# dome272/Paella

Hardware: AMD Instinct MI355X
Metric: images/sec (whole node) + single-image ms, 256x256 @ 8 steps (higher is better)
Workload: dtype f32; 1 GPU; BASELINE configs[1]: Paella 573M-class (stand-in blocks=[4,8,4]) (570.3M params), 32x32 tokens = 256 px, 8 steps, CFG 8.0, CLIP-H-text only (S=4), batch 1 per GPU, + VQGAN f8 decode; denoiser=570m, sample_steps=8, noise=philox, submission=hip-graph replay, world_size_observed=1

## Files before the change

paella_amd/_lib.py:

```python
import ctypes
import os
from ctypes import POINTER, Structure, c_char, c_char_p, c_float, c_int, c_int32, c_int64, c_size_t, c_uint64, c_void_p

_HERE = os.path.dirname(os.path.abspath(__file__))
LIB_PATH = os.path.join(_HERE, "csrc", "libpaella_hip.so")

MAX_LEVELS = 8
MAX_BLOCK_TYPES = 8
ABI_VERSION = 8


class UnetConfig(Structure):
    _fields_ = [
        ("c_in", c_int32), ("c_out", c_int32), ("num_labels", c_int32), ("c_r", c_int32), ("patch_size", c_int32),
        ("c_cond", c_int32), ("n_levels", c_int32),
        ("c_hidden", c_int32 * MAX_LEVELS), ("nhead", c_int32 * MAX_LEVELS), ("blocks", c_int32 * MAX_LEVELS),
        ("level_config", (c_char * MAX_BLOCK_TYPES) * MAX_LEVELS),
        ("clip_embd", c_int32), ("byt5_embd", c_int32), ("clip_seq_len", c_int32), ("kernel_size", c_int32),
        ("self_attn", c_int32),
    ]


class VqganConfig(Structure):
    _fields_ = [
# ... 208 lines not shown
    "paella_test_attention_bf16_ragged": (c_int, [c_void_p, c_void_p, c_void_p, c_void_p, c_void_p, c_void_p, c_int, c_int, c_int, c_int, c_int, c_int, c_void_p,
                                                  c_void_p, c_int, c_void_p]),
    "paella_test_attention_bf16_kw": (c_int, [c_void_p, c_void_p, c_void_p, c_void_p, c_void_p, c_void_p, c_int, c_int, c_int, c_int, c_int, c_int, c_void_p,
                                              c_void_p, c_void_p, c_int, c_void_p]),
    "paella_test_launch_chain": (c_int, [c_void_p, c_int, c_int, c_int, c_void_p]),
    "paella_test_attention_variant": (c_int, [c_int]),
    "paella_test_gemm_dma": (c_int, [c_int]),
    "paella_test_gemm_epi_specialise": (c_int, [c_int]),
    "paella_test_gemm_raster": (c_int, [c_int]),
    "paella_test_gemm_ring": (c_int, [c_int]),
    "paella_test_ring_resident": (ctypes.c_long, [c_int, c_int]),
    "paella_test_gemm_site": (c_int, [c_int, c_int, c_int, c_int, c_int, c_int]),
    "paella_test_gemm_site_cfg": (c_int, [c_int, c_int, c_int, c_int, c_int, c_int, c_int]),
    "paella_test_gemm_big_stagger": (c_int, [c_int]),
    "paella_test_grn_fuse": (c_int, [c_int]),
    "paella_test_ln_fold_ratio": (c_int, [c_float]),
    "paella_test_ln_guard_counter": (c_int, [c_void_p]),
    "paella_test_mlp_grn_fused": (c_int, [c_void_p] * 10 + [c_int, c_int, c_int, c_void_p, c_size_t, c_void_p]),
    "paella_test_gemm_tail_tile": (c_int, [c_int]),
    "paella_test_tail_scores": (c_int, [c_void_p, c_void_p, c_int64, c_int, c_float, c_float, c_float, c_uint64, c_uint64, c_int64, c_void_p, c_void_p]),
    "paella_test_tail_scores_req": (c_int, [c_void_p, c_void_p, c_int64, c_int, c_void_p, c_void_p, c_void_p, c_int, c_uint64, c_void_p, c_void_p]),
    "paella_test_tail_filter_keep": (c_int, [c_void_p, c_void_p, c_int64, c_int, c_float, c_float, c_float, c_int, c_float, c_float, c_int, c_void_p, c_void_p, c_void_p,
                                             c_int, c_void_p, c_void_p, c_void_p, c_void_p, c_void_p]),
    "paella_test_renoise_scores": (c_int, [c_void_p, c_void_p, c_void_p, c_int64, c_int, c_uint64, c_uint64, c_int64, c_float, c_int, c_float, c_void_p, c_void_p, c_void_p,
                                           c_void_p, c_void_p, c_void_p, c_void_p, c_void_p, c_void_p, c_void_p, c_void_p, c_void_p]),
    "paella_test_gemm_prologue": (c_int, [c_void_p, c_void_p, c_void_p, c_int, c_int, c_int, c_int, c_void_p, c_void_p, c_int, c_void_p, c_int, c_int,
                                          c_void_p, c_size_t, c_void_p]),
    "paella_test_gemm_desc": (c_int, [POINTER(TestGemmArgs), c_int, c_int, c_void_p, c_size_t, c_void_p]),
    "paella_test_gemm_args_size": (c_size_t, []),
}
# ... 63 lines not shown
```

paella_amd/csrc/common.h:

```cpp
#pragma once
#include <hip/hip_runtime.h>
#include <stdint.h>
#include <stddef.h>

typedef float f32x4 __attribute__((ext_vector_type(4)));

#define PAELLA_OK 0
#define PAELLA_ERR_ARG -1
#define PAELLA_ERR_HIP -2
#define PAELLA_ERR_WORKSPACE -3
#define PAELLA_ERR_STATE -4

void paella_set_error(const char* fmt, ...);

#define HIP_CHECK_RET(expr)                                                          \
    do {                                                                             \
        hipError_t _e = (expr);                                                      \
        if (_e != hipSuccess) {                                                      \
            paella_set_error("%s:%d: %s -> %s", __FILE__, __LINE__, #expr,           \
                             hipGetErrorString(_e));                                 \
            return PAELLA_ERR_HIP;                                                   \
        }                                                                            \
    } while (0)

// ... 97 lines not shown
    int M, N, K;
    const float* a_scale;
    const float* a_shift;
    int a_rows_per_sample;
    FastDiv a_rps_div;
    const float* grn_gx;
    const float* grn_gamma;
    const float* grn_part;
    int grn_np;
    int force_ring_cfg;
    const float* ln_stats;
    int ln_nblk;
    float ln_eps;
    const float* ln_row;
    float ln_fold_ratio;
    const float* ln_wsum;
    unsigned* ln_guard_count;
    Epilogue ep;
    FusedTail ft;
    ConvGather cv;
    const unsigned short* A16;
    const unsigned short* W16;
    ReqTables rq;
};

struct TailArgs;
static const size_t kGemmMaxTickets = (size_t)1 << 16;
static const size_t kGemmTicketBytes = kGemmMaxTickets * sizeof(unsigned);
int launch_gemm(const GemmArgs& g, void* ws, size_t ws_bytes, hipStream_t stream);
int launch_gemm_cfg(const GemmArgs& g, int cfg, int splitk, void* ws, size_t ws_bytes, hipStream_t stream);
// ... 135 lines not shown
```

paella_amd/csrc/gemm.hip:

```cpp
#include "common.h"
#include "gemm_device.h"
#include "philox.h"
#include <stdio.h>
#include <stdlib.h>
#include "test_hooks.h"
#include <atomic>
#include <mutex>
#include <string>
#include <type_traits>
#include <utility>
#include <vector>

typedef unsigned int u32x4 __attribute__((ext_vector_type(4)));
typedef __bf16 bf16x8 __attribute__((ext_vector_type(8)));

template <typename F, int... Is>
__device__ __forceinline__ void static_for_impl(F& f, std::integer_sequence<int, Is...>) { (f(std::integral_constant<int, Is>{}), ...); }
template <int N, typename F>
__device__ __forceinline__ void static_for(F& f) { static_for_impl(f, std::make_integer_sequence<int, N>{}); }

struct SkPlan {
    int tiles_m, tiles_n;
    int KT;
    unsigned U;
// ... 71 lines not shown
constexpr int tile_wg_per_cu(int WM, int WN, int TM, int TN, int PD, int APRO, bool TAIL, int BK, bool DMA, int RING, bool BF) {
    const int NW = WM * WN, blocks = TM * TN;
    if (RING > 0) {
        const int wish = NW == 8 ? 1 : blocks == 1 ? (RING == 3 ? 5 : 4) : (blocks == 2 ? ((BF && APRO == 2 && TM == 2) ? 3 : 4) : 3);
        const int fit = (160 * 1024) / tile_res(WM, WN, TM, TN, APRO, TAIL, BK, RING).lds_bytes;
        return fit < wish ? (fit < 1 ? 1 : fit) : wish;
    }
    if (TAIL && DMA) return 4;
    if (TAIL && NW == 8 && blocks == 4) return 4;
    if (WM == 2 && WN == 2 && blocks == 1 && PD == 2 && BK == 32 && (APRO == 0 || APRO == 3)) return 5;
    if (DMA && NW == 4 && blocks == 16) return 2;
    if (NW == 8 && WM * TM == 8 && WN * TN == 4 && PD == 2 && BK == 32 && APRO == 0 && !TAIL) return 4;
    return 1;
}

template <int WM, int WN, int TM, int TN, int PD, int APRO, bool TAIL = false, int BK = 32, bool DMA = false, int RING = 0, bool BF = false, int EPI = EPI_RUNTIME, bool REQ = false>
__global__ __launch_bounds__(64 * WM * WN, tile_wg_per_cu(WM, WN, TM, TN, PD, APRO, TAIL, BK, DMA, RING, BF)) void gemm_nt_kernel(GemmArgs g, SkPlan p, float* __restrict__ slabs,
                                                               unsigned* __restrict__ tickets, unsigned slab_bytes) {
    constexpr TileRes RES = tile_res(WM, WN, TM, TN, APRO, TAIL, BK, RING);
    constexpr int BM = RES.BM, BN = RES.BN;
    constexpr int SL = BK / 4;
    constexpr int KG = BK / 16;
    constexpr int NW = WM * WN, NT = 64 * NW;
    constexpr int RP = NT / SL;
    constexpr int LA = (BM * SL + NT - 1) / NT, LB = (BN * SL + NT - 1) / NT;
    static_assert(NW == 4 || NW == 8, "4 or 8 waves per workgroup");
    static_assert(!REQ || TAIL, "the request form exists for the fused tail only");
    static_assert(PD == 1 || PD == 2, "prefetch ring depth 1 or 2");
    static_assert(BK == 32 || BK == 64, "K step of 32 or 64");
    static_assert(!BF || ((DMA || RING > 0) && (APRO == 0 || APRO == 2) && BK == 32), "bf16 operands: direct-to-LDS / ring variants, no operand transform");
    constexpr int ESZ = BF ? 2 : 4;
    constexpr bool DMA_W = DMA || RING > 0, DMA_A = (DMA && (APRO == 0 || APRO == 2)) || RING > 0;
    static_assert(!DMA || (PD == 1 && BK == 32 && (BM * SL) % NT == 0 && (BN * SL) % NT == 0), "DMA variant: 1-deep, K step 32, whole passes");
    constexpr bool PP = RING == 2;
    static_assert(!PP || (BF && NW == 8 && WM == 2 && WN == 4 && TM == 8 && TN == 4 && (APRO == 0 || APRO == 2)), "ping-pong tile: bf16 operands, 2 x 4 waves of 128x64 wave tiles");
    static_assert(RING == 0 || (RING >= 2 && RING <= 4 && !DMA && PD == 1 && BK == 32 && !TAIL && APRO != 3 && (NW == 4 || (TM == 4 && TN == 4 && RING == 3) || PP) && (BM * SL) % NT == 0 && (BN * SL) % NT == 0),
                  "ring variant: 3 or 4 LDS stages (2 for the ping-pong tile), 4 waves (or 8 waves of 64x64 / 128x64 wave tiles), K step 32, whole passes, no implicit convolution");
    static_assert(APRO != 4 || RING > 0, "the GRN-from-raw-statistics prologue exists on ring tiles only");
    constexpr bool BIG = RING > 0 && NW == 8;
    static_assert(!BIG || APRO != 4, "the 8-wave ring tile has no GRN-from-raw-statistics prologue");
    constexpr bool GRN_SIDE = RING > 0 && (APRO == 1 || APRO == 4);
    constexpr bool GRN_FIN = RING > 0 && !BIG;
    constexpr int TILE_FLOATS = RES.tile_floats, STAGE_FLOATS = RES.stage_floats, FLAG_OFF = RES.flag_off, TAIL_FLOATS = RES.tail_floats;
    static_assert(RES.side_samples == (BIG ? 16 : 8) && (RES.grn_scr > 0) == GRN_FIN, "tile_res() and the kernel agree on which ring tiles are BIG");
    __shared__ __attribute__((aligned(16))) float smem[RES.lds_bytes / 4];

    const unsigned G = p.G;
    unsigned gid = blockIdx.x;
    {
        const unsigned q = G >> 3, r = G & 7;
        const unsigned xcd = gid & 7, idx = gid >> 3;
        gid = xcd * q + min(xcd, r) + idx;
    }
    const unsigned u0 = sk_start(p, gid);
    const int n = (int)(p.q + (gid < p.r ? 1u : 0u));
// ... 27 lines not shown
    };
    Stage R[PD];

    int ltile = (int)fast_div(u0, p.dKT);
    int lkt = (int)(u0 - (unsigned)ltile * (unsigned)KT);
    auto rsrc_of = [](const void* ptr, size_t bytes) {
        return __builtin_amdgcn_make_buffer_rsrc(const_cast<void*>(ptr), 0, (int)(bytes > 0xffffffffull ? 0xffffffffull : bytes), 0x00020000);
    };
    const char* const Abase = BF ? reinterpret_cast<const char*>(g.A16) : reinterpret_cast<const char*>(g.A);
    const char* const Wbase = BF ? reinterpret_cast<const char*>(g.W16) : reinterpret_cast<const char*>(g.W);
    const size_t a_bytes = APRO == 3 ? (size_t)(g.M / (g.cv.Ho * g.cv.Wo)) * g.cv.Hi * g.cv.Wi * g.cv.C * sizeof(float)
                                     : ((size_t)(g.M - 1) * g.lda + g.K) * ESZ;
    const size_t w_bytes = ((size_t)(g.N - 1) * g.ldw + g.K) * ESZ;
    __amdgpu_buffer_rsrc_t rsrcA = rsrc_of(Abase, a_bytes), rsrcW = rsrc_of(Wbase, w_bytes);
    __amdgpu_buffer_rsrc_t rsrcS = rsrc_of(g.A, 16);
    const __amdgpu_buffer_rsrc_t rsrcT = rsrc_of((APRO == 1 || APRO == 4) ? g.a_shift : g.A, (APRO == 1 || APRO == 4) ? (size_t)g.K * sizeof(float) : 16);
    const __amdgpu_buffer_rsrc_t rsrcG = rsrc_of(APRO == 4 ? g.grn_gamma : g.A, APRO == 4 ? (size_t)g.K * sizeof(float) : 16);
    unsigned aoff[LA], soff[APRO == 1 ? LA : 1], boff[LB];
    unsigned aux_s_off2 = 0;
    unsigned aux_s_off = 0;
    int cy[APRO == 3 ? LA : 1], cx[APRO == 3 ? LA : 1];
    int ltap = 0, lc0 = 0;
    auto set_tile = [&](int tile) __attribute__((always_inline)) {
        int tile_m, tile_n;
        sk_tile_coords<(BM >= 64)>(p, tile, tile_m, tile_n);
        const int m0 = tile_m * BM, n0 = tile_n * BN;
        size_t a_base;
        int img0 = 0, smp0 = 0;
        if (APRO == 3) {
            img0 = m0 / (g.cv.Ho * g.cv.Wo);
            a_base = (size_t)img0 * g.cv.Hi * g.cv.Wi * g.cv.C * sizeof(float);
// ... 189 lines not shown
                a = __builtin_bit_cast(f32x4, __builtin_shufflevector(lo, hi, 0, 1, 2, 3, 4, 5, 6, 7));
            }
        }
    };
    int kt_cur = 0;

    auto load_unit = [&](Stage& r, int dma_slot) __attribute__((always_inline)) {
        float* dAs = smem + dma_slot * (RING > 0 ? STAGE_FLOATS : TILE_FLOATS) + (wave * (64 / SL)) * BK;
        float* dBs = dAs + BM * BK;
        const int kofs = lkt * (BK * 4);
        if constexpr (RING > 0) {
#pragma unroll
            for (int i = 0; i < LA; ++i) dma_b128_to_lds(rsrcA, dAs + i * RP * BK, aoff[i], kofs);
#pragma unroll
            for (int i = 0; i < LB; ++i) dma_b128_to_lds<((BIG || TM * TN != 1) ? 0 : PAELLA_RING_W_AUX)>(rsrcW, dBs + i * RP * BK, boff[i], kofs);
            if (GRN_SIDE && wave == NW - 1) {
                float* dX = smem + dma_slot * STAGE_FLOATS + TILE_FLOATS;
                if (BIG) {
                    if (lane_k < 8) dma_b128_to_lds(rsrcT, dX, (unsigned)(lane_k * 16), kofs);
                    dma_b128_to_lds(rsrcS, dX + 64, aux_s_off, kofs);
                    dma_b128_to_lds(rsrcS, dX + 64 + 256, aux_s_off2, kofs);
                } else if (APRO == 4) {
                    if (lane_k < 8) {
                        dma_b128_to_lds(rsrcT, dX, (unsigned)(lane_k * 16), kofs);
                        dma_b128_to_lds(rsrcG, dX + 32, (unsigned)(lane_k * 16), kofs);
                    }
                    dma_b128_to_lds(rsrcS, dX + 64, aux_s_off, kofs);
                } else {
                    dma_b128_to_lds(rsrcT, dX, (unsigned)((lane_k & 7) * 16), kofs);
                    dma_b128_to_lds(rsrcS, dX + 256, aux_s_off, kofs);
                }
            }
            return;
        }
        int oy = 0, ox = 0;
        if (APRO == 3) {
            oy = g.cv.oy0 + g.cv.tsign * (ltap >> g.cv.tw_log2);
            ox = g.cv.ox0 + g.cv.tsign * (ltap & ((1 << g.cv.tw_log2) - 1));
        }
#pragma unroll
        for (int i = 0; i < LA; ++i) {
            if (APRO == 3) {
                const int yy = cy[i] + oy, xx = cx[i] + ox;
                r.ok[i] = (unsigned)yy < (unsigned)g.cv.Hi && (unsigned)xx < (unsigned)g.cv.Wi;
// ... 486 lines not shown
                    const int row = (wn * TN + j) * 16 + r16;
                    bf[kk][j] = *reinterpret_cast<const f32x4*>(Bs + row * BK + ((c4 ^ (row & (SL - 1))) << 2));
                }
            }
            if (APRO == 2 && ln_any) {
#pragma unroll
                for (int kk = 0; kk < KG; ++kk)
#pragma unroll
                    for (int i = 0; i < TM; ++i) ln_fix(af[kk][i], i, BF_FIX ? kt_ring * BK + (kk * 4 + kq) * 4 : 0);
            }
            if (APRO == 1) {
                const float* X = Bs + BN * BK;
#pragma unroll
                for (int kk = 0; kk < KG; ++kk) {
                    const int c4 = kk * 4 + kq;
                    const f32x4 t = *reinterpret_cast<const f32x4*>(X + c4 * 4);
#pragma unroll
                    for (int i = 0; i < TM; ++i) {
                        const f32x4 sc = *reinterpret_cast<const f32x4*>(X + 256 + sidx[i] * 32 + c4 * 4);
                        af[kk][i] = af[kk][i] * sc + t;
                    }
                }
            }
            if (APRO == 4) {
                const float* X = Bs + BN * BK;
#pragma unroll
                for (int kk = 0; kk < KG; ++kk) {
                    const int c4 = kk * 4 + kq;
                    const f32x4 t = *reinterpret_cast<const f32x4*>(X + c4 * 4);
                    const f32x4 gm = *reinterpret_cast<const f32x4*>(X + 32 + c4 * 4);
#pragma unroll
                    for (int i = 0; i < TM; ++i) {
                        const f32x4 gx = *reinterpret_cast<const f32x4*>(X + 64 + sidx[i] * 32 + c4 * 4);
                        const f32x4 sc = gm * gx * rinv[i] + 1.0f;
                        af[kk][i] = af[kk][i] * sc + t;
                    }
                }
            }
            if constexpr (BF) {
                if (TM * TN == 1) {
#pragma unroll
                    for (int kk = 0; kk < KG; kk += 2) {
                        acc[0][0] = mma_bf16(bf[kk][0], af[kk][0], acc[0][0]);
                        acc2 = mma_bf16(bf[kk + 1][0], af[kk + 1][0], acc2);
                    }
                } else {
#pragma unroll
                    for (int kk = 0; kk < KG; ++kk)
#pragma unroll
                        for (int i = 0; i < TM; ++i)
// ... 19 lines not shown
                            for (int j = 0; j < TN; ++j)
                                acc[i][j] = __builtin_amdgcn_mfma_f32_16x16x4f32(bf[kk][j][e], af[kk][i][e], acc[i][j], 0, 0, 0);
            }
        };
        auto fetch_ring = [&](int stage) __attribute__((always_inline)) {
            load_unit(R[0], stage);
            if (++loaded < n) {
                if (++lkt == KT) {
                    lkt = 0;
                    ++ltile;
                    set_tile(ltile);
                }
            }
        };
        constexpr int PER_UNIT = LA + LB;
        constexpr int SIDE_DMAS = (APRO == 4 || BIG) ? 3 : 2;
        if constexpr (PP) {
            using I0 = std::integral_constant<int, 0>;
            using I1 = std::integral_constant<int, 1>;
            using I2 = std::integral_constant<int, 2>;
            using I3 = std::integral_constant<int, 3>;
            using I4 = std::integral_constant<int, 4>;
            int lbuf = 0;
            auto pp_issue = [&](auto sec_tag) __attribute__((always_inline)) {
                constexpr int sec = decltype(sec_tag)::value;
                float* dAs = smem + lbuf * STAGE_FLOATS + (wave * (64 / SL)) * BK;
                float* dBs = dAs + BM * BK;
                const int kofs = lkt * (BK * 4);
                if constexpr (sec == 0) {
                    dma_b128_to_lds(rsrcA, dAs, aoff[0], kofs);
                    dma_b128_to_lds(rsrcA, dAs + 2 * RP * BK, aoff[2], kofs);
// ... 193 lines not shown
                __builtin_amdgcn_sched_barrier(0);
                if (i + seg_len == n) asm volatile("s_waitcnt vmcnt(0)" ::: "memory");
                if (first_seg) ln_row_stats();
                flush(ctile, ckt, ckt + seg_len, first_seg);
                first_seg = false;
                i += seg_len;
                ckt += seg_len;
                if (ckt == KT) { ckt = 0; ++ctile; }
            }
            return;
        }
        for (int i = 0; i < n;) {
            const int seg_len = min(KT - ckt, n - i);
            enter_tile(ctile);
            for (int s2 = 0; s2 < seg_len; ++s2) {
                if (GRN_SIDE && wave == NW - 1) asm volatile("s_waitcnt vmcnt(%0)" ::"n"((RING - 2) * (PER_UNIT + SIDE_DMAS)) : "memory");
                else asm volatile("s_waitcnt vmcnt(%0)" ::"n"((RING - 2) * PER_UNIT) : "memory");
                __builtin_amdgcn_s_barrier();
                asm volatile("" ::: "memory");
                fetch_ring(ls);
                __builtin_amdgcn_sched_barrier(0);
                compute_ring(cs, ckt + s2);
                __builtin_amdgcn_sched_barrier(0);
                cs = cs + 1 == RING ? 0 : cs + 1;
                ls = ls + 1 == RING ? 0 : ls + 1;
            }
            if (i + seg_len == n) asm volatile("s_waitcnt vmcnt(0)" ::: "memory");
            flush(ctile, ckt, ckt + seg_len, first_seg);
            first_seg = false;
            i += seg_len;
            ckt += seg_len;
// ... 193 lines not shown
};
template <int APRO> struct RingEpi { using set = EpiSet<>; };
template <> struct RingEpi<0> { using set = EpiSet<EPI_B, EPI_BGF, EPI_BGS, EPI_BR, EPI_BRS>; };
template <> struct RingEpi<1> { using set = EpiSet<EPI_BR, EPI_BRS, EPI_BRT, EPI_BRST>; };
template <> struct RingEpi<2> { using set = EpiSet<EPI_B>; };
template <> struct RingEpi<4> { using set = EpiSet<EPI_BR, EPI_BRS, EPI_BRT, EPI_BRST>; };

struct Launch {
    const GemmArgs& g;
    const SkPlan& p;
    float* slabs;
    unsigned* tickets;
    unsigned slab_bytes;
    hipStream_t st;
};
template <int ID, int APRO, bool TAIL = false, bool DMA = false, int RING = 0, bool BF = false, int EPI = EPI_RUNTIME, bool REQ = false>
static void launch_kernel(const Launch& l) {
    constexpr Tile t = kCfgs[ID];
    hipLaunchKernelGGL((gemm_nt_kernel<t.wm, t.wn, t.tm, t.tn, t.pd, APRO, TAIL, t.bk, DMA, RING, BF, EPI, REQ>), dim3(l.p.G), dim3(64 * t.waves()), 0, l.st, l.g, l.p, l.slabs,
                       l.tickets, l.slab_bytes);
}

template <int ID, int APRO, int EPI>
static bool launch_ring_if(int cls, const Launch& l) {
    if (cls != EPI) return false;
    launch_kernel<ID, APRO, false, false, kCfgs[ID].ring, false, EPI>(l);
    g_last_epi = EPI;
    return true;
}
template <int ID, int APRO, int... C>
static void launch_ring_epi(EpiSet<C...>, const Launch& l) {
    const int cls = g_gemm_epi_spec ? epi_class(l.g) : EPI_RUNTIME;
    if (!(launch_ring_if<ID, APRO, C>(cls, l) || ...)) launch_ring_if<ID, APRO, EPI_RUNTIME>(EPI_RUNTIME, l);
}
template <int ID, int APRO>
static void launch_ring_apro(const Launch& l) {
    using set = typename std::conditional<kCfgs[ID].tm * kCfgs[ID].tn == 1, typename RingEpi<APRO>::set, EpiSet<>>::type;
    launch_ring_epi<ID, APRO>(set{}, l);
}
template <int ID>
static void launch_ring(const Launch& l) {
    if (l.g.grn_gx) launch_ring_apro<ID, 4>(l);
    else if (l.g.a_scale) launch_ring_apro<ID, 1>(l);
    else if (l.g.ln_stats) launch_ring_apro<ID, 2>(l);
    else launch_ring_apro<ID, 0>(l);
}

template <int ID>
static void launch_one(const Launch& l) {
    constexpr Tile t = kCfgs[ID];
    const GemmArgs& g = l.g;
    if constexpr (t.has(V_DMA | V_DMA_PLAIN)) {
        if (g_gemm_dma && g.K % t.bk == 0 && !g.cv.enabled && !g.a_scale && !g.ln_stats) return launch_kernel<ID, 0, false, true>(l);
// ... 284 lines not shown
    g_prof.shape.insert(g_prof.shape.end(), shp, shp + 5);
    return rc;
}

static std::atomic<float> g_ln_fold_ratio{kLnFoldMaxRatio};
extern "C" int paella_test_ln_fold_ratio(float ratio) { g_ln_fold_ratio = ratio; return PAELLA_OK; }
static std::atomic<unsigned*> g_ln_guard_count{nullptr};
extern "C" int paella_test_ln_guard_counter(unsigned* dev_word) { g_ln_guard_count = dev_word; return PAELLA_OK; }

int launch_gemm_cfg(const GemmArgs& g_in, int cfg, int splitk, void* ws, size_t ws_bytes, hipStream_t st) {
    GemmArgs g = g_in;
    g.ln_fold_ratio = g_ln_fold_ratio.load(std::memory_order_relaxed);
    g.ln_guard_count = g_ln_guard_count.load(std::memory_order_relaxed);
    g.a_rps_div = fast_div_of((unsigned)(g.a_rows_per_sample > 0 ? g.a_rows_per_sample : 1));
    g.ep.rps_div = fast_div_of((unsigned)(g.ep.rows_per_sample > 0 ? g.ep.rows_per_sample : 1));
    return prof_bracket(g, st, true, [&]() { return launch_gemm_cfg_impl(g, cfg, splitk, ws, ws_bytes, st); });
}

extern "C" int paella_prof_enable(int on) {
    std::lock_guard<std::mutex> lock(g_prof_mu);
    g_prof.on = on != 0;
    g_prof.used = 0;
    g_prof.flops.clear();
    g_prof.bytes.clear();
    g_prof.shape.clear();
    g_prof.epi.clear();
    g_prof.grid.clear();
    return PAELLA_OK;
}

// ... 149 lines not shown
        if (bf && cfg_has(cfg, V_BF16) && g.ln_stats && !g.ln_row && !prepass_fits && bf16_ln_needs_prepass(cfg, g.A != nullptr)) {
            cfg = 18;
            if (splitk >= 0) G = (unsigned)(tiles_of_cfg(cfg, g.M, g.N) * (splitk < 1 ? 1 : splitk));
        }
    }
    const Tile& tc = kCfgs[cfg];
    const int BM = tc.res().BM, BN = tc.res().BN;
    g_last_cfg = cfg;
    if (bf && g.ln_stats && !g.ln_row && bf16_ln_needs_prepass(cfg, g.A != nullptr)) {
        if (!prepass_fits) { paella_set_error("internal: bf16 LayerNorm-consuming launch on tile %d without room for its row pre-pass", cfg); return PAELLA_ERR_STATE; }
        const int rc = ln_prepass();
        if (rc != PAELLA_OK) return rc;
    }
    if (bf && !cfg_has(cfg, V_BF16)) { paella_set_error("gemm: tile config %d has no bf16-operand variant (%s do)", cfg, ids_with(V_BF16).c_str()); return PAELLA_ERR_ARG; }
    if ((g.grn_gx || g.ep.grn_gx_out) && (!tc.ring || tc.waves() == 8)) { paella_set_error("gemm: the in-epilogue / on-load GRN statistics need a ring tile (got tile %d)", cfg); return PAELLA_ERR_STATE; }
    if (g.grn_gx && (!g.grn_gamma || !g.a_shift || !g.grn_part || g.grn_np <= 0 || g.a_scale || g.ln_stats || g.a_rows_per_sample % 16)) {
        paella_set_error("gemm: bad GRN-from-statistics operand description"); return PAELLA_ERR_ARG;
    }
    if (g.ep.grn_gx_out && (!g.ep.grn_part_out || !(g.ep.grn_rps == 16 || g.ep.grn_rps == BM) || g.M % g.ep.grn_rps ||
                            g.ep.grn_np != ((g.N + BN - 1) / BN) * tc.wn)) {
        paella_set_error("gemm: in-epilogue GRN needs tiles that cover whole samples (rows per sample 16 or %d, got %d) and grn_np = tiles_n * %d", BM, g.ep.grn_rps, tc.wn);
        return PAELLA_ERR_ARG;
    }
    if (tc.ring && !ring_ok(g, cfg)) { paella_set_error("gemm: tile config %d (LDS-DMA ring) needs K %% 32 == 0, no implicit convolution and <= 8 samples per tile", cfg); return PAELLA_ERR_ARG; }
    SkPlan p;
    unsigned slab_bytes = 0;
    const int rc = make_plan("gemm", g, cfg, bf, G, g_gemm_big_stagger.load(std::memory_order_relaxed), have_ws, slab_cap, p, slab_bytes);
    if (rc != PAELLA_OK) return rc;
    const Launch l{g, p, have_ws ? reinterpret_cast<float*>(reinterpret_cast<char*>(ws) + kGemmTicketBytes) : nullptr, have_ws ? reinterpret_cast<unsigned*>(ws) : nullptr, slab_bytes, st};
    if (!launch_tile(TileIds{}, cfg, bf, l)) { paella_set_error("gemm: tile config %d (%dx%d) exists for bf16 operands only", cfg, BM, BN); return PAELLA_ERR_ARG; }
    LAUNCH_CHECK_RET();
// ... 80 lines not shown
```

paella_amd/csrc/internal.h:

```cpp
#pragma once
#include "common.h"
#include "../../include/paella_hip.h"
#include <vector>

#define RET_IF(expr)                      \
    do {                                  \
        int _rc = (expr);                 \
        if (_rc != PAELLA_OK) return _rc; \
    } while (0)

struct DevBuf {
    float* p = nullptr;
    size_t n = 0;
    bool loaded = false;
};
int devbuf_alloc(DevBuf& b, size_t n);
struct DevBuf16 {
    unsigned short* p = nullptr;
    size_t n = 0;
};

struct Arena {
    char* base;
    size_t cap, off;
// ... 34 lines not shown
    return t;
}
static inline paella_tail_args tail_block_stream(const float* logits_c, const float* logits_u, int64_t rows, int L, const float* cfg_pairs, const float* temperature,
                                                 const uint64_t* seeds, int rows_per_sample, const int* step, const float* t_next, const int* active, const int64_t* init_noise,
                                                 const int64_t* pin_keep, const int64_t* pin_tokens, const int* pin_on, int64_t* tokens_out, int64_t* sampled_out) {
    paella_tail_args t = {};
    t.logits_c = logits_c; t.logits_u = logits_u; t.rows = rows; t.L = L; t.cfg_pairs = cfg_pairs; t.temperature_tab = temperature; t.seeds = seeds;
    t.rows_per_sample = rows_per_sample; t.step = step; t.t_next_tab = t_next; t.active = active; t.init_noise = init_noise;
    t.pin_keep = pin_keep; t.pin_tokens = pin_tokens; t.pin_on = pin_on; t.tokens_out = tokens_out; t.sampled_out = sampled_out;
    return t;
}

static inline GemmArgs gemm_args(const float* A, int lda, const float* Wt, int ldw, float* C, int ldc, int M, int N, int K) {
    GemmArgs g;
    g.A = A; g.lda = lda; g.W = Wt; g.ldw = ldw; g.C = C; g.ldc = ldc; g.M = M; g.N = N; g.K = K;
    g.a_scale = nullptr; g.a_shift = nullptr; g.a_rows_per_sample = 1; g.a_rps_div.mul = 0; g.a_rps_div.shr = 0; g.a_rps_div.pass = 0xffffffffu; g.grn_gx = nullptr; g.grn_gamma = nullptr; g.grn_part = nullptr; g.grn_np = 0; g.force_ring_cfg = 0; g.ln_stats = nullptr; g.ln_nblk = 0; g.ln_eps = 1e-6f; g.ln_wsum = nullptr; g.ln_row = nullptr; g.ln_fold_ratio = 4.0f; g.ln_guard_count = nullptr;
    g.ep = make_epilogue();
    g.ft.temperature = 1.f; g.ft.mode = 0; g.ft.seed = 0; g.ft.seed_ptr = nullptr; g.ft.offset = 0; g.ft.row_offset = 0; g.ft.row_offset_ptr = nullptr;
    g.ft.part_score = nullptr; g.ft.part_idx = nullptr;
    g.cv.enabled = 0;
    g.A16 = nullptr; g.W16 = nullptr;
    return g;
}
```

paella_amd/csrc/model.hip:

```cpp
#include "internal.h"
#include "test_hooks.h"
#include "../../include/paella_hip.h"

#include <math.h>
#include <stdarg.h>
#include <stdio.h>
#include <string.h>

#include <map>
#include <string>
#include <vector>

static thread_local char g_err[2048] = "";
void paella_set_error(const char* fmt, ...) {
    va_list ap;
    va_start(ap, fmt);
    vsnprintf(g_err, sizeof(g_err), fmt, ap);
    va_end(ap);
}
extern "C" const char* paella_last_error(void) { return g_err; }
extern "C" int paella_abi_version(void) { return PAELLA_ABI_VERSION; }

int devbuf_alloc(DevBuf& b, size_t n) {
    if (b.p && b.n == n) return PAELLA_OK;
// ... 22 lines not shown
    int fused_ts = -1;
    int attn_index = -1;
    bool emit_rowstat = false;
    bool ln_from_stats = false;
    int c_from = 0, c_to = 0;
};

struct paella_unet {
    paella_unet_config cfg;
    std::vector<Block> down, up;
    std::map<std::string, TensorSpec> specs;
    std::map<std::string, DevBuf> t;
    DevBuf ts_w, ts_b, freqs;
    DevBuf kv_w, kv_b;
    std::map<std::string, DevBuf> wsum;
    int precision = 0;
    std::map<std::string, DevBuf16> t16;
    std::map<std::string, DevBuf> wsum16;
    std::vector<int> kv_col;
    int kv_total = 0;
    int ts_total = 0;
    int n_attn = 0;
    std::vector<int> attn_c;
    bool finalized = false;
    bool freqs_set = false;
    bool clf_from_stats = false;
    int c_max = 0;
};

static const float* T(const paella_unet* m, const std::string& k) {
// ... 168 lines not shown
    if (rc != PAELLA_OK) { delete m; return rc; }
    if (m->ts_total > 0) {
        rc = devbuf_alloc(m->ts_w, (size_t)m->ts_total * cfg->c_r);
        if (rc == PAELLA_OK) rc = devbuf_alloc(m->ts_b, (size_t)m->ts_total);
        if (rc != PAELLA_OK) { delete m; return rc; }
    }
    *out = m;
    return PAELLA_OK;
}

extern "C" void paella_unet_destroy(paella_unet* m) {
    if (!m) return;
    for (auto& kv : m->t) if (kv.second.p) (void)hipFree(kv.second.p);
    for (auto& kv : m->wsum) if (kv.second.p) (void)hipFree(kv.second.p);
    for (auto& kv : m->wsum16) if (kv.second.p) (void)hipFree(kv.second.p);
    for (auto& kv : m->t16) if (kv.second.p) (void)hipFree(kv.second.p);
    if (m->kv_w.p) (void)hipFree(m->kv_w.p);
    if (m->kv_b.p) (void)hipFree(m->kv_b.p);
    if (m->ts_w.p) (void)hipFree(m->ts_w.p);
    if (m->ts_b.p) (void)hipFree(m->ts_b.p);
    if (m->freqs.p) (void)hipFree(m->freqs.p);
    delete m;
}

int repack_into(Repack kind, const float* src, const std::vector<int64_t>& shape, DevBuf& dst, hipStream_t st) {
    int64_t numel = 1;
    for (int64_t d : shape) numel *= d;
    switch (kind) {
        case RP_COPY:
            RET_IF(devbuf_alloc(dst, numel));
// ... 128 lines not shown
        RET_IF(devbuf_alloc(dst, (size_t)t.second.first));
        RET_IF(launch_rowsum_bf16(it->second.p, dst.p, t.second.first, t.second.second, st));
    }
    HIP_CHECK_RET(hipStreamSynchronize(st));
    return PAELLA_OK;
}

extern "C" int paella_unet_set_precision(paella_unet* m, int mode, void* stream) {
    if (!m) { paella_set_error("null argument"); return PAELLA_ERR_ARG; }
    if (mode != 0 && mode != 1) { paella_set_error("precision mode must be 0 (fp32) or 1 (bf16 operands)"); return PAELLA_ERR_ARG; }
    m->precision = mode;
    if (mode == 1 && m->finalized) return make_shadows(m, (hipStream_t)stream);
    return PAELLA_OK;
}
extern "C" int paella_unet_get_precision(const paella_unet* m) { return m ? m->precision : 0; }

extern "C" int paella_unet_finalize(paella_unet* m, void* stream) {
    if (!m) { paella_set_error("null argument"); return PAELLA_ERR_ARG; }
    for (auto& kv : m->specs) {
        auto it = m->t.find(kv.first);
        if (it == m->t.end() || !it->second.loaded) { paella_set_error("tensor '%s' was never loaded", kv.first.c_str()); return PAELLA_ERR_STATE; }
    }
    {
        hipStream_t st = (hipStream_t)stream;
        std::vector<std::pair<std::string, std::pair<int, int>>> todo;
        auto want = [&](const Block& b) {
            if (b.type == BT_ATTN && b.ln_from_stats) todo.push_back({b.prefix + ".attention.attn.in_proj_weight", {3 * b.c, b.c}});
            if (b.type == BT_UP && b.ln_from_stats) todo.push_back({b.prefix + ".1.weight", {4 * b.c_to, b.c_from}});
        };
        for (const Block& b : m->down) want(b);
// ... 41 lines not shown
            const int perm[2] = {1, 0};
            RET_IF(launch_permute(T(m, b.prefix + ".kv_mapper.1.weight"), wkv_t.p, shp, perm, 2, st));
            GemmArgs g = gemm_args(win, ch, wkv_t.p, ch, m->kv_w.p + (size_t)m->kv_col[b.attn_index] * cc, cc, 2 * ch, cc, ch);
            RET_IF(launch_gemm_cfg(g, 18, 1, nullptr, 0, st));
            GemmArgs gb = gemm_args(T(m, b.prefix + ".kv_mapper.1.bias"), ch, win, ch, m->kv_b.p + m->kv_col[b.attn_index], 2 * ch, 1, 2 * ch, ch);
            gb.ep.bias = bin;
            RET_IF(launch_gemm_cfg(gb, 5, 1, nullptr, 0, st));
            return PAELLA_OK;
        };
        if (rc == PAELLA_OK) for (const Block& b : m->down) { rc = compose(b); if (rc != PAELLA_OK) break; }
        if (rc == PAELLA_OK) for (const Block& b : m->up) { rc = compose(b); if (rc != PAELLA_OK) break; }
        if (hipStreamSynchronize(st) != hipSuccess && rc == PAELLA_OK) { paella_set_error("finalize: stream error while composing the conditioning projections"); rc = PAELLA_ERR_HIP; }
        if (wkv_t.p) (void)hipFree(wkv_t.p);
        if (rc != PAELLA_OK) return rc;
    }
    if (!m->freqs_set) {
        const int half = m->cfg.c_r / 2;
        std::vector<float> f(half > 0 ? half : 1);
        const float e = logf(10000.0f) / (float)(half - 1);
        for (int k = 0; k < half; ++k) f[k] = expf((float)k * -e);
        RET_IF(paella_unet_set_timestep_freqs(m, f.data(), half));
    }
    m->finalized = true;
    if (m->precision == 1) RET_IF(make_shadows(m, (hipStream_t)stream));
    return PAELLA_OK;
}

extern "C" size_t paella_unet_cond_bytes(const paella_unet* m, int B, int S) {
    if (!m) return 0;
    const size_t n = (size_t)B * S * (size_t)m->kv_total;
// ... 204 lines not shown
        g2.A16 = cx.f.g16; g2.W16 = w2_16;
        g2.ep.bias = T(m, b.prefix + ".channelwise.4.bias");
        g2.ep.residual = x; g2.ep.ldr = ch;
        g2.ep.c16 = x16;
        if (b.emit_rowstat) g2.ep.rowstat_out = cx.f.rowstat;
        if (b.fused_ts >= 0) {
            g2.ep.ts = cx.f.ts + b.fused_ts; g2.ep.ts_stride = m->ts_total; g2.ep.rows_per_sample = rps;
        }
        RET_IF(launch_gemm(g2, cx.f.splitk, kSplitKBudget, cx.st));
        return PAELLA_OK;
    }
    if (b.type == BT_RES)
        RET_IF(launch_dwconv_ln(x, skip, T(m, b.prefix + ".depthwise.weight"), T(m, b.prefix + ".depthwise.bias"), cx.f.h, cx.B, h, w, ch, 1e-6f, cx.st));
    else
        RET_IF(launch_layernorm(x, cx.f.h, rows, ch, 1e-6f, 1.f, 0.f, 0, 0, 0, cx.st));
    GemmArgs g1 = gemm_args(cx.f.h, ch, T(m, b.prefix + ".channelwise.0.weight"), ch, cx.f.g, 4 * ch, (int)rows, 4 * ch, ch);
    g1.ep.bias = T(m, b.prefix + ".channelwise.0.bias");
    g1.ep.act = ACT_GELU;
    const int fused_tile = (rps % 16 == 0 && m->precision == 0) ? gemm_grn_fused_tile((int)rows, 4 * ch, ch, rps, false) : 0;
    if (fused_tile) {
        const int np = (4 * ch / 32) * 2;
        g1.ep.grn_gx_out = cx.f.grn_scale; g1.ep.grn_part_out = cx.f.grn_gx; g1.ep.grn_rps = rps; g1.ep.grn_np = np;
        g1.force_ring_cfg = fused_tile;
        RET_IF(launch_gemm(g1, cx.f.splitk, kSplitKBudget, cx.st));
        GemmArgs g2 = gemm_args(cx.f.g, 4 * ch, T(m, b.prefix + ".channelwise.4.weight"), 4 * ch, x, ch, (int)rows, ch, 4 * ch);
        g2.grn_gx = cx.f.grn_scale; g2.grn_part = cx.f.grn_gx; g2.grn_np = np; g2.grn_gamma = T(m, b.prefix + ".channelwise.2.gamma");
        g2.a_shift = T(m, b.prefix + ".channelwise.2.beta");
        g2.a_rows_per_sample = rps;
        g2.ep.bias = T(m, b.prefix + ".channelwise.4.bias");
        g2.ep.residual = x; g2.ep.ldr = ch;
        if (b.emit_rowstat) g2.ep.rowstat_out = cx.f.rowstat;
        if (b.fused_ts >= 0) {
            g2.ep.ts = cx.f.ts + b.fused_ts; g2.ep.ts_stride = m->ts_total; g2.ep.rows_per_sample = rps;
        }
        RET_IF(launch_gemm(g2, cx.f.splitk, kSplitKBudget, cx.st));
        return PAELLA_OK;
    }
    if (rps % 16 == 0) {
        g1.ep.sumsq_out = cx.f.grn_gx;
        RET_IF(launch_gemm(g1, cx.f.splitk, kSplitKBudget, cx.st));
        RET_IF(launch_grn_from_partials(cx.f.grn_gx, T(m, b.prefix + ".channelwise.2.gamma"), cx.f.grn_scale, cx.B, rps / 16, 4 * ch, cx.st));
    } else {
        RET_IF(launch_gemm(g1, cx.f.splitk, kSplitKBudget, cx.st));
        RET_IF(launch_grn_scale(cx.f.g, T(m, b.prefix + ".channelwise.2.gamma"), cx.f.grn_scale, cx.f.grn_gx, cx.B, rps, 4 * ch, cx.st));
    }
    GemmArgs g2 = gemm_args(cx.f.g, 4 * ch, T(m, b.prefix + ".channelwise.4.weight"), 4 * ch, x, ch, (int)rows, ch, 4 * ch);
    g2.a_scale = cx.f.grn_scale;
    g2.a_shift = T(m, b.prefix + ".channelwise.2.beta");
    g2.a_rows_per_sample = rps;
    g2.ep.bias = T(m, b.prefix + ".channelwise.4.bias");
    g2.ep.residual = x; g2.ep.ldr = ch;
    g2.ep.c16 = x16;
    if (b.emit_rowstat) g2.ep.rowstat_out = cx.f.rowstat;
    if (b.fused_ts >= 0) {
        g2.ep.ts = cx.f.ts + b.fused_ts; g2.ep.ts_stride = m->ts_total; g2.ep.rows_per_sample = rps;
    }
    RET_IF(launch_gemm(g2, cx.f.splitk, kSplitKBudget, cx.st));
    return PAELLA_OK;
}

static int run_attn_block(FwdCtx& cx, const Block& b, float* x, int h, int w) {
    const paella_unet* m = cx.m;
    const int ch = b.c;
    const int64_t rows = (int64_t)cx.B * h * w;
    const int nh = m->cfg.nhead[b.level];
// ... 701 lines not shown
```

Baseline: 47.19 images/sec.

## Fold GRN beta shift into second MLP GEMM bias at finalize

```diff
diff --git a/paella_amd/_lib.py b/paella_amd/_lib.py
--- a/paella_amd/_lib.py
+++ b/paella_amd/_lib.py
@@ -246,6 +246,9 @@
     "paella_test_gemm_site_cfg": (c_int, [c_int, c_int, c_int, c_int, c_int, c_int, c_int]),
     "paella_test_gemm_big_stagger": (c_int, [c_int]),
     "paella_test_grn_fuse": (c_int, [c_int]),
+    "paella_test_grn_shift_fold": (c_int, [c_int]),
+    "paella_test_gemm_noshift": (c_int, [c_int]),
+    "paella_test_gemm_noshift_launches": (c_int64, []),
     "paella_test_ln_fold_ratio": (c_int, [c_float]),
     "paella_test_ln_guard_counter": (c_int, [c_void_p]),
     "paella_test_mlp_grn_fused": (c_int, [c_void_p] * 10 + [c_int, c_int, c_int, c_void_p, c_size_t, c_void_p]),
diff --git a/paella_amd/csrc/common.h b/paella_amd/csrc/common.h
--- a/paella_amd/csrc/common.h
+++ b/paella_amd/csrc/common.h
@@ -135,6 +135,7 @@
     float ln_eps;
     const float* ln_row;
     float ln_fold_ratio;
+    unsigned a_shift_bytes;
     const float* ln_wsum;
     unsigned* ln_guard_count;
     Epilogue ep;
diff --git a/paella_amd/csrc/gemm.hip b/paella_amd/csrc/gemm.hip
--- a/paella_amd/csrc/gemm.hip
+++ b/paella_amd/csrc/gemm.hip
@@ -109,7 +109,7 @@
     return 1;
 }
 
-template <int WM, int WN, int TM, int TN, int PD, int APRO, bool TAIL = false, int BK = 32, bool DMA = false, int RING = 0, bool BF = false, int EPI = EPI_RUNTIME, bool REQ = false>
+template <int WM, int WN, int TM, int TN, int PD, int APRO, bool TAIL = false, int BK = 32, bool DMA = false, int RING = 0, bool BF = false, int EPI = EPI_RUNTIME, bool REQ = false, bool NOSHIFT = false>
 __global__ __launch_bounds__(64 * WM * WN, tile_wg_per_cu(WM, WN, TM, TN, PD, APRO, TAIL, BK, DMA, RING, BF)) void gemm_nt_kernel(GemmArgs g, SkPlan p, float* __restrict__ slabs,
                                                                unsigned* __restrict__ tickets, unsigned slab_bytes) {
     constexpr TileRes RES = tile_res(WM, WN, TM, TN, APRO, TAIL, BK, RING);
@@ -134,6 +134,9 @@
     static_assert(APRO != 4 || RING > 0, "the GRN-from-raw-statistics prologue exists on ring tiles only");
     constexpr bool BIG = RING > 0 && NW == 8;
     static_assert(!BIG || APRO != 4, "the 8-wave ring tile has no GRN-from-raw-statistics prologue");
+    static_assert(!NOSHIFT || (RING > 0 && !BIG && (APRO == 1 || APRO == 4)), "the shift-free form exists for the GRN prologues of the 4-wave ring tiles");
+    constexpr bool SIDE_SPREAD = NOSHIFT && APRO == 4;
+    constexpr bool SHIFT = (APRO == 1 || APRO == 4) && !NOSHIFT;
     constexpr bool GRN_SIDE = RING > 0 && (APRO == 1 || APRO == 4);
     constexpr bool GRN_FIN = RING > 0 && !BIG;
     constexpr int TILE_FLOATS = RES.tile_floats, STAGE_FLOATS = RES.stage_floats, FLAG_OFF = RES.flag_off, TAIL_FLOATS = RES.tail_floats;
@@ -191,7 +194,7 @@
     const size_t w_bytes = ((size_t)(g.N - 1) * g.ldw + g.K) * ESZ;
     __amdgpu_buffer_rsrc_t rsrcA = rsrc_of(Abase, a_bytes), rsrcW = rsrc_of(Wbase, w_bytes);
     __amdgpu_buffer_rsrc_t rsrcS = rsrc_of(g.A, 16);
-    const __amdgpu_buffer_rsrc_t rsrcT = rsrc_of((APRO == 1 || APRO == 4) ? g.a_shift : g.A, (APRO == 1 || APRO == 4) ? (size_t)g.K * sizeof(float) : 16);
+    const __amdgpu_buffer_rsrc_t rsrcT = rsrc_of(SHIFT ? g.a_shift : g.A, !SHIFT ? 16 : APRO == 1 ? (size_t)g.a_shift_bytes : (size_t)g.K * sizeof(float));
     const __amdgpu_buffer_rsrc_t rsrcG = rsrc_of(APRO == 4 ? g.grn_gamma : g.A, APRO == 4 ? (size_t)g.K * sizeof(float) : 16);
     unsigned aoff[LA], soff[APRO == 1 ? LA : 1], boff[LB];
     unsigned aux_s_off2 = 0;
@@ -411,7 +414,13 @@
             for (int i = 0; i < LA; ++i) dma_b128_to_lds(rsrcA, dAs + i * RP * BK, aoff[i], kofs);
 #pragma unroll
             for (int i = 0; i < LB; ++i) dma_b128_to_lds<((BIG || TM * TN != 1) ? 0 : PAELLA_RING_W_AUX)>(rsrcW, dBs + i * RP * BK, boff[i], kofs);
-            if (GRN_SIDE && wave == NW - 1) {
+            if constexpr (SIDE_SPREAD) {
+                float* dX = smem + dma_slot * STAGE_FLOATS + TILE_FLOATS;
+                if (wave == NW - 2) {
+                    if (lane_k < 8) dma_b128_to_lds(rsrcG, dX + 32, (unsigned)(lane_k * 16), kofs);
+                }
+                if (wave == NW - 1) dma_b128_to_lds(rsrcS, dX + 64, aux_s_off, kofs);
+            } else if (GRN_SIDE && wave == NW - 1) {
                 float* dX = smem + dma_slot * STAGE_FLOATS + TILE_FLOATS;
                 if (BIG) {
                     if (lane_k < 8) dma_b128_to_lds(rsrcT, dX, (unsigned)(lane_k * 16), kofs);
@@ -419,12 +428,12 @@
                     dma_b128_to_lds(rsrcS, dX + 64 + 256, aux_s_off2, kofs);
                 } else if (APRO == 4) {
                     if (lane_k < 8) {
-                        dma_b128_to_lds(rsrcT, dX, (unsigned)(lane_k * 16), kofs);
+                        if (!NOSHIFT) dma_b128_to_lds(rsrcT, dX, (unsigned)(lane_k * 16), kofs);
                         dma_b128_to_lds(rsrcG, dX + 32, (unsigned)(lane_k * 16), kofs);
                     }
                     dma_b128_to_lds(rsrcS, dX + 64, aux_s_off, kofs);
                 } else {
-                    dma_b128_to_lds(rsrcT, dX, (unsigned)((lane_k & 7) * 16), kofs);
+                    if (!NOSHIFT) dma_b128_to_lds(rsrcT, dX, (unsigned)((lane_k & 7) * 16), kofs);
                     dma_b128_to_lds(rsrcS, dX + 256, aux_s_off, kofs);
                 }
             }
@@ -941,11 +950,13 @@
 #pragma unroll
                 for (int kk = 0; kk < KG; ++kk) {
                     const int c4 = kk * 4 + kq;
-                    const f32x4 t = *reinterpret_cast<const f32x4*>(X + c4 * 4);
+                    f32x4 t;
+                    if constexpr (!NOSHIFT) t = *reinterpret_cast<const f32x4*>(X + c4 * 4);
 #pragma unroll
                     for (int i = 0; i < TM; ++i) {
                         const f32x4 sc = *reinterpret_cast<const f32x4*>(X + 256 + sidx[i] * 32 + c4 * 4);
-                        af[kk][i] = af[kk][i] * sc + t;
+                        if constexpr (NOSHIFT) af[kk][i] = af[kk][i] * sc;
+                        else af[kk][i] = af[kk][i] * sc + t;
                     }
                 }
             }
@@ -954,13 +965,15 @@
 #pragma unroll
                 for (int kk = 0; kk < KG; ++kk) {
                     const int c4 = kk * 4 + kq;
-                    const f32x4 t = *reinterpret_cast<const f32x4*>(X + c4 * 4);
+                    f32x4 t;
+                    if constexpr (!NOSHIFT) t = *reinterpret_cast<const f32x4*>(X + c4 * 4);
                     const f32x4 gm = *reinterpret_cast<const f32x4*>(X + 32 + c4 * 4);
 #pragma unroll
                     for (int i = 0; i < TM; ++i) {
                         const f32x4 gx = *reinterpret_cast<const f32x4*>(X + 64 + sidx[i] * 32 + c4 * 4);
                         const f32x4 sc = gm * gx * rinv[i] + 1.0f;
-                        af[kk][i] = af[kk][i] * sc + t;
+                        if constexpr (NOSHIFT) af[kk][i] = af[kk][i] * sc;
+                        else af[kk][i] = af[kk][i] * sc + t;
                     }
                 }
             }
@@ -1010,7 +1023,7 @@
             }
         };
         constexpr int PER_UNIT = LA + LB;
-        constexpr int SIDE_DMAS = (APRO == 4 || BIG) ? 3 : 2;
+        constexpr int SIDE_DMAS = ((APRO == 4 || BIG) ? 3 : 2) - (NOSHIFT ? 1 : 0);
         if constexpr (PP) {
             using I0 = std::integral_constant<int, 0>;
             using I1 = std::integral_constant<int, 1>;
@@ -1234,7 +1247,8 @@
             const int seg_len = min(KT - ckt, n - i);
             enter_tile(ctile);
             for (int s2 = 0; s2 < seg_len; ++s2) {
-                if (GRN_SIDE && wave == NW - 1) asm volatile("s_waitcnt vmcnt(%0)" ::"n"((RING - 2) * (PER_UNIT + SIDE_DMAS)) : "memory");
+                if (SIDE_SPREAD && wave >= NW - 2) asm volatile("s_waitcnt vmcnt(%0)" ::"n"((RING - 2) * (PER_UNIT + 1)) : "memory");
+                else if (!SIDE_SPREAD && GRN_SIDE && wave == NW - 1) asm volatile("s_waitcnt vmcnt(%0)" ::"n"((RING - 2) * (PER_UNIT + SIDE_DMAS)) : "memory");
                 else asm volatile("s_waitcnt vmcnt(%0)" ::"n"((RING - 2) * PER_UNIT) : "memory");
                 __builtin_amdgcn_s_barrier();
                 asm volatile("" ::: "memory");
@@ -1458,29 +1472,41 @@
     unsigned slab_bytes;
     hipStream_t st;
 };
-template <int ID, int APRO, bool TAIL = false, bool DMA = false, int RING = 0, bool BF = false, int EPI = EPI_RUNTIME, bool REQ = false>
+template <int ID, int APRO, bool TAIL = false, bool DMA = false, int RING = 0, bool BF = false, int EPI = EPI_RUNTIME, bool REQ = false, bool NOSHIFT = false>
 static void launch_kernel(const Launch& l) {
     constexpr Tile t = kCfgs[ID];
-    hipLaunchKernelGGL((gemm_nt_kernel<t.wm, t.wn, t.tm, t.tn, t.pd, APRO, TAIL, t.bk, DMA, RING, BF, EPI, REQ>), dim3(l.p.G), dim3(64 * t.waves()), 0, l.st, l.g, l.p, l.slabs,
+    hipLaunchKernelGGL((gemm_nt_kernel<t.wm, t.wn, t.tm, t.tn, t.pd, APRO, TAIL, t.bk, DMA, RING, BF, EPI, REQ, NOSHIFT>), dim3(l.p.G), dim3(64 * t.waves()), 0, l.st, l.g, l.p, l.slabs,
                        l.tickets, l.slab_bytes);
 }
 
-template <int ID, int APRO, int EPI>
+static std::atomic<int> g_gemm_noshift{1};
+static std::atomic<long long> g_gemm_noshift_launches{0};
+extern "C" int paella_test_gemm_noshift(int on) { g_gemm_noshift = on != 0; return PAELLA_OK; }
+extern "C" long long paella_test_gemm_noshift_launches(void) { return g_gemm_noshift_launches.load(); }
+
+template <int ID, int APRO, int EPI, bool NOSHIFT>
 static bool launch_ring_if(int cls, const Launch& l) {
     if (cls != EPI) return false;
-    launch_kernel<ID, APRO, false, false, kCfgs[ID].ring, false, EPI>(l);
+    launch_kernel<ID, APRO, false, false, kCfgs[ID].ring, false, EPI, false, NOSHIFT>(l);
     g_last_epi = EPI;
+    if (NOSHIFT) ++g_gemm_noshift_launches;
     return true;
 }
-template <int ID, int APRO, int... C>
+template <int ID, int APRO, bool NOSHIFT, int... C>
 static void launch_ring_epi(EpiSet<C...>, const Launch& l) {
     const int cls = g_gemm_epi_spec ? epi_class(l.g) : EPI_RUNTIME;
-    if (!(launch_ring_if<ID, APRO, C>(cls, l) || ...)) launch_ring_if<ID, APRO, EPI_RUNTIME>(EPI_RUNTIME, l);
+    if (!(launch_ring_if<ID, APRO, C, NOSHIFT>(cls, l) || ...)) launch_ring_if<ID, APRO, EPI_RUNTIME, NOSHIFT>(EPI_RUNTIME, l);
 }
 template <int ID, int APRO>
 static void launch_ring_apro(const Launch& l) {
-    using set = typename std::conditional<kCfgs[ID].tm * kCfgs[ID].tn == 1, typename RingEpi<APRO>::set, EpiSet<>>::type;
-    launch_ring_epi<ID, APRO>(set{}, l);
+    constexpr bool small = kCfgs[ID].tm * kCfgs[ID].tn == 1;
+    using set = typename std::conditional<small, typename RingEpi<APRO>::set, EpiSet<>>::type;
+    if constexpr (APRO == 4) {
+        if (!l.g.a_shift_bytes) return launch_ring_epi<ID, APRO, true>(set{}, l);
+    } else if constexpr (small && APRO == 1) {
+        if (!l.g.a_shift_bytes && g_gemm_noshift) return launch_ring_epi<ID, APRO, true>(set{}, l);
+    }
+    launch_ring_epi<ID, APRO, false>(set{}, l);
 }
 template <int ID>
 static void launch_ring(const Launch& l) {
@@ -1795,6 +1821,8 @@
     g.ln_guard_count = g_ln_guard_count.load(std::memory_order_relaxed);
     g.a_rps_div = fast_div_of((unsigned)(g.a_rows_per_sample > 0 ? g.a_rows_per_sample : 1));
     g.ep.rps_div = fast_div_of((unsigned)(g.ep.rows_per_sample > 0 ? g.ep.rows_per_sample : 1));
+    g.a_shift_bytes = g.a_shift ? (unsigned)g.K * (unsigned)sizeof(float) : 0u;
+    if (!g.a_shift) g.a_shift = g.A;
     return prof_bracket(g, st, true, [&]() { return launch_gemm_cfg_impl(g, cfg, splitk, ws, ws_bytes, st); });
 }
 
@@ -1974,7 +2002,7 @@
     }
     if (bf && !cfg_has(cfg, V_BF16)) { paella_set_error("gemm: tile config %d has no bf16-operand variant (%s do)", cfg, ids_with(V_BF16).c_str()); return PAELLA_ERR_ARG; }
     if ((g.grn_gx || g.ep.grn_gx_out) && (!tc.ring || tc.waves() == 8)) { paella_set_error("gemm: the in-epilogue / on-load GRN statistics need a ring tile (got tile %d)", cfg); return PAELLA_ERR_STATE; }
-    if (g.grn_gx && (!g.grn_gamma || !g.a_shift || !g.grn_part || g.grn_np <= 0 || g.a_scale || g.ln_stats || g.a_rows_per_sample % 16)) {
+    if (g.grn_gx && (!g.grn_gamma || !g.grn_part || g.grn_np <= 0 || g.a_scale || g.ln_stats || g.a_rows_per_sample % 16)) {
         paella_set_error("gemm: bad GRN-from-statistics operand description"); return PAELLA_ERR_ARG;
     }
     if (g.ep.grn_gx_out && (!g.ep.grn_part_out || !(g.ep.grn_rps == 16 || g.ep.grn_rps == BM) || g.M % g.ep.grn_rps ||
diff --git a/paella_amd/csrc/internal.h b/paella_amd/csrc/internal.h
--- a/paella_amd/csrc/internal.h
+++ b/paella_amd/csrc/internal.h
@@ -72,7 +72,7 @@
 static inline GemmArgs gemm_args(const float* A, int lda, const float* Wt, int ldw, float* C, int ldc, int M, int N, int K) {
     GemmArgs g;
     g.A = A; g.lda = lda; g.W = Wt; g.ldw = ldw; g.C = C; g.ldc = ldc; g.M = M; g.N = N; g.K = K;
-    g.a_scale = nullptr; g.a_shift = nullptr; g.a_rows_per_sample = 1; g.a_rps_div.mul = 0; g.a_rps_div.shr = 0; g.a_rps_div.pass = 0xffffffffu; g.grn_gx = nullptr; g.grn_gamma = nullptr; g.grn_part = nullptr; g.grn_np = 0; g.force_ring_cfg = 0; g.ln_stats = nullptr; g.ln_nblk = 0; g.ln_eps = 1e-6f; g.ln_wsum = nullptr; g.ln_row = nullptr; g.ln_fold_ratio = 4.0f; g.ln_guard_count = nullptr;
+    g.a_scale = nullptr; g.a_shift = nullptr; g.a_shift_bytes = 0; g.a_rows_per_sample = 1; g.a_rps_div.mul = 0; g.a_rps_div.shr = 0; g.a_rps_div.pass = 0xffffffffu; g.grn_gx = nullptr; g.grn_gamma = nullptr; g.grn_part = nullptr; g.grn_np = 0; g.force_ring_cfg = 0; g.ln_stats = nullptr; g.ln_nblk = 0; g.ln_eps = 1e-6f; g.ln_wsum = nullptr; g.ln_row = nullptr; g.ln_fold_ratio = 4.0f; g.ln_guard_count = nullptr;
     g.ep = make_epilogue();
     g.ft.temperature = 1.f; g.ft.mode = 0; g.ft.seed = 0; g.ft.seed_ptr = nullptr; g.ft.offset = 0; g.ft.row_offset = 0; g.ft.row_offset_ptr = nullptr;
     g.ft.part_score = nullptr; g.ft.part_idx = nullptr;
diff --git a/paella_amd/csrc/model.hip b/paella_amd/csrc/model.hip
--- a/paella_amd/csrc/model.hip
+++ b/paella_amd/csrc/model.hip
@@ -7,6 +7,7 @@
 #include <stdio.h>
 #include <string.h>
 
+#include <atomic>
 #include <map>
 #include <string>
 #include <vector>
@@ -60,6 +61,8 @@
     DevBuf ts_w, ts_b, freqs;
     DevBuf kv_w, kv_b;
     std::map<std::string, DevBuf> wsum;
+    std::map<std::string, DevBuf> b2f;
+    bool grn_shift_fold = true;
     int precision = 0;
     std::map<std::string, DevBuf16> t16;
     std::map<std::string, DevBuf> wsum16;
@@ -258,6 +261,7 @@
     for (auto& kv : m->t) if (kv.second.p) (void)hipFree(kv.second.p);
     for (auto& kv : m->wsum) if (kv.second.p) (void)hipFree(kv.second.p);
     for (auto& kv : m->wsum16) if (kv.second.p) (void)hipFree(kv.second.p);
+    for (auto& kv : m->b2f) if (kv.second.p) (void)hipFree(kv.second.p);
     for (auto& kv : m->t16) if (kv.second.p) (void)hipFree(kv.second.p);
     if (m->kv_w.p) (void)hipFree(m->kv_w.p);
     if (m->kv_b.p) (void)hipFree(m->kv_b.p);
@@ -416,6 +420,9 @@
     return PAELLA_OK;
 }
 extern "C" int paella_unet_get_precision(const paella_unet* m) { return m ? m->precision : 0; }
+
+static std::atomic<int> g_grn_shift_fold{1};
+extern "C" int paella_test_grn_shift_fold(int on) { g_grn_shift_fold = on != 0; return PAELLA_OK; }
 
 extern "C" int paella_unet_finalize(paella_unet* m, void* stream) {
     if (!m) { paella_set_error("null argument"); return PAELLA_ERR_ARG; }
@@ -487,6 +494,24 @@
         if (wkv_t.p) (void)hipFree(wkv_t.p);
         if (rc != PAELLA_OK) return rc;
     }
+    {
+        hipStream_t st = (hipStream_t)stream;
+        m->grn_shift_fold = g_grn_shift_fold.load(std::memory_order_relaxed) != 0;
+        int rc = PAELLA_OK;
+        auto fold = [&](const Block& b) -> int {
+            if (b.type != BT_RES && b.type != BT_FF) return PAELLA_OK;
+            const int ch = b.c;
+            DevBuf& dst = m->b2f[b.prefix];
+            RET_IF(devbuf_alloc(dst, (size_t)ch));
+            GemmArgs g = gemm_args(T(m, b.prefix + ".channelwise.2.beta"), 4 * ch, T(m, b.prefix + ".channelwise.4.weight"), 4 * ch, dst.p, ch, 1, ch, 4 * ch);
+            g.ep.bias = T(m, b.prefix + ".channelwise.4.bias");
+            return launch_gemm_cfg(g, 5, 1, nullptr, 0, st);
+        };
+        for (const Block& b : m->down) { rc = fold(b); if (rc != PAELLA_OK) break; }
+        if (rc == PAELLA_OK) for (const Block& b : m->up) { rc = fold(b); if (rc != PAELLA_OK) break; }
+        if (hipStreamSynchronize(st) != hipSuccess && rc == PAELLA_OK) { paella_set_error("finalize: stream error while folding the GRN shifts"); rc = PAELLA_ERR_HIP; }
+        if (rc != PAELLA_OK) return rc;
+    }
     if (!m->freqs_set) {
         const int half = m->cfg.c_r / 2;
         std::vector<float> f(half > 0 ? half : 1);
@@ -721,6 +746,7 @@
         RET_IF(launch_dwconv_ln(x, skip, T(m, b.prefix + ".depthwise.weight"), T(m, b.prefix + ".depthwise.bias"), cx.f.h, cx.B, h, w, ch, 1e-6f, cx.st));
     else
         RET_IF(launch_layernorm(x, cx.f.h, rows, ch, 1e-6f, 1.f, 0.f, 0, 0, 0, cx.st));
+    const bool fold = m->grn_shift_fold;
     GemmArgs g1 = gemm_args(cx.f.h, ch, T(m, b.prefix + ".channelwise.0.weight"), ch, cx.f.g, 4 * ch, (int)rows, 4 * ch, ch);
     g1.ep.bias = T(m, b.prefix + ".channelwise.0.bias");
     g1.ep.act = ACT_GELU;
@@ -732,9 +758,9 @@
         RET_IF(launch_gemm(g1, cx.f.splitk, kSplitKBudget, cx.st));
         GemmArgs g2 = gemm_args(cx.f.g, 4 * ch, T(m, b.prefix + ".channelwise.4.weight"), 4 * ch, x, ch, (int)rows, ch, 4 * ch);
         g2.grn_gx = cx.f.grn_scale; g2.grn_part = cx.f.grn_gx; g2.grn_np = np; g2.grn_gamma = T(m, b.prefix + ".channelwise.2.gamma");
-        g2.a_shift = T(m, b.prefix + ".channelwise.2.beta");
+        g2.a_shift = fold ? nullptr : T(m, b.prefix + ".channelwise.2.beta");
         g2.a_rows_per_sample = rps;
-        g2.ep.bias = T(m, b.prefix + ".channelwise.4.bias");
+        g2.ep.bias = fold ? m->b2f.at(b.prefix).p : T(m, b.prefix + ".channelwise.4.bias");
         g2.ep.residual = x; g2.ep.ldr = ch;
         if (b.emit_rowstat) g2.ep.rowstat_out = cx.f.rowstat;
         if (b.fused_ts >= 0) {
@@ -753,9 +779,9 @@
     }
     GemmArgs g2 = gemm_args(cx.f.g, 4 * ch, T(m, b.prefix + ".channelwise.4.weight"), 4 * ch, x, ch, (int)rows, ch, 4 * ch);
     g2.a_scale = cx.f.grn_scale;
-    g2.a_shift = T(m, b.prefix + ".channelwise.2.beta");
+    g2.a_shift = fold ? nullptr : T(m, b.prefix + ".channelwise.2.beta");
     g2.a_rows_per_sample = rps;
-    g2.ep.bias = T(m, b.prefix + ".channelwise.4.bias");
+    g2.ep.bias = fold ? m->b2f.at(b.prefix).p : T(m, b.prefix + ".channelwise.4.bias");
     g2.ep.residual = x; g2.ep.ldr = ch;
     g2.ep.c16 = x16;
     if (b.emit_rowstat) g2.ep.rowstat_out = cx.f.rowstat;
```

Measured after the change: 47.59 images/sec, median of 6. Within noise of the previous version (+0.9%).
